# MyrtleSoftware/myrtlespeech

Hardware: AMD Instinct MI355X
Metric: audio-sec/s (RTF), DS2 5xBiLSTM-1024 encoder forward + CTC greedy, 80-feature 10 s clips @ batch 32/GPU (higher is better)
Workload: dtype f16x3 (f32 split in fp16 hi+lo, 3 fp16 MFMA passes, f32 acc: LSTM, projections, conv1/2, FC1; FC2/CTC/decode f32)

## Files before the change

### include/ms_hotpath.h

```cpp
#ifndef MS_HOTPATH_H
#define MS_HOTPATH_H

#include <stddef.h>
#include <stdint.h>

#ifdef __cplusplus
extern "C" {
#endif

#define MS_ABI_VERSION 4

enum {
  MS_OK = 0,
  MS_ERR_INVALID = 1,
  MS_ERR_HIP = 2,
  MS_ERR_WORKSPACE = 3,
  MS_ERR_TIMEOUT = 4,
  MS_ERR_UNSUPPORTED = 5
};

enum { MS_CELL_LSTM = 0, MS_CELL_GRU = 1, MS_CELL_RNN_TANH = 2, MS_CELL_HARD_LSTM = 3 };

enum { MS_ACT_NONE = 0, MS_ACT_CLAMP = 1  };

// ... 21 lines not shown
                           void* workspace, size_t workspace_bytes, void* stream);

size_t ms_maskconv_fwin_packed_bytes(int Cout, int KF, int KT);
int ms_maskconv_fwin_pack(const float* w, void* packed, int Cout, int KF, int KT, void* stream);
size_t ms_maskconv_fwin_workspace_bytes(int N, int Tin, int KF, int SF, int Fout);
int ms_maskconv_fwin_forward(const float* x, const int32_t* lens, const void* packed_w, const float* bias, float* y, int N,
                             int Fin, int Tin, int Cout, int Fout, int Tout, int KF, int KT, int SF, int ST, int DT,
                             int pad_f_l, int pad_t_l, int act, float act_lo, float act_hi, void* workspace,
                             size_t workspace_bytes, void* stream);

size_t ms_maskconv1d_gemm_packed_bytes(int Cout, int Cin, int KT);
int ms_maskconv1d_gemm_pack(const float* w, void* packed, int Cout, int Cin, int KT, void* stream);
size_t ms_maskconv1d_gemm_workspace_bytes(int N, int Cin, int Tout, int Cout, int KT);
int ms_maskconv1d_gemm_forward(const float* x, const int32_t* lens, const void* packed, const float* bias, float* y, int N,
                               int Cin, int Tin, int Cout, int Tout, int KT, int ST, int DT, int pad_l, int act,
                               float act_lo, float act_hi, void* workspace, size_t workspace_bytes, void* stream);

int ms_nct_to_tnc(const float* x, float* y, int N, int CF, int T, void* stream);

int ms_clamp(const float* x, float* y, size_t n, float lo, float hi, void* stream);


int ms_linear_forward(const float* x, const float* w, const float* bias, float* y, int M, int K, int N, int act,
                      float act_lo, float act_hi, void* stream);

#define MS_LINEAR_FEW_ROWS 1
size_t ms_linear_splitk_workspace_bytes(int M, int K, int N, int flags);
int ms_linear_splitk_forward(const float* x, const float* w, const float* bias, float* y, int M, int K, int N, int act,
                             float act_lo, float act_hi, int flags, void* workspace, size_t workspace_bytes, void* stream);

size_t ms_linear_split_workspace_bytes(int M, int K, int N);
int ms_linear_split_forward(const float* x, const float* w, const float* bias, float* y, int M, int K, int N, int act,
                            float act_lo, float act_hi, void* workspace, size_t workspace_bytes, void* stream);

size_t ms_linear_split_packed_bytes(int K, int N);
int ms_linear_split_pack(const float* w, void* packed, int K, int N, void* stream);
int ms_linear_split_forward_packed(const float* x, const void* packed_w, const float* bias, float* y, int M, int K, int N, int act,
                                   float act_lo, float act_hi, void* workspace, size_t workspace_bytes, void* stream);


int ms_lookahead_forward(const float* x, const float* w, float* y, int N, int F, int T, int ctx, long xs_n,
                         long xs_f, long xs_t, long ys_n, long ys_f, long ys_t, int act, float act_lo,
                         float act_hi, void* stream);

int ms_lookahead_window_forward(const float* x, const float* w, float* y, int N, int F, int T_in, int T_out, int ctx,
                                long xs_n, long xs_f, long xs_t, long ys_n, long ys_f, long ys_t, int act, float act_lo,
                                float act_hi, void* stream);


int ms_rnn_padded_hidden(int cell, int H, int ndir);
size_t ms_rnn_packed_bytes(int cell, int In, int H, int ndir);
int ms_rnn_pack(int cell, int In, int H, int ndir, const float* const* w_ih_host, const float* const* w_hh_host,
                const float* const* b_ih_host, const float* const* b_hh_host, void* packed, void* stream);

size_t ms_rnn_workspace_bytes(int cell, int T, int N, int In, int H, int ndir);

int ms_rnn_layer_forward(int cell, const void* packed, const float* x, const int32_t* lens, int max_len,
                         const float* h0, const float* c0, float* out, float* hn, float* cn, int T, int N, int In,
                         int H, int ndir, void* workspace, size_t workspace_bytes, void* stream);

enum { MS_RNN_X_PLANES_IN_WS = 1, MS_RNN_OUT_PLANES_TO_WS = 2, MS_RNN_PACKED_ROWS = 4, MS_RNN_HX_PREINIT = 4096,
       MS_RNN_RECURRENCE_ONLY = 8192, MS_RNN_TIMING_SKIP_PROJECTION = 8192 ,
       MS_RNN_PROJECTION_ONLY = 16384 };
int ms_rnn_layer_chains_planes(int cell, int H, int ndir);
int ms_rnn_hx_preinit(int cell, int T, int N, int In, int H, int ndir, int max_len, int nregions, void* workspace,
                      size_t workspace_bytes, void* stream);
int ms_rnn_layer_packs_rows(int cell, int T, int N, int In, int H, int ndir);
int ms_rnn_layer_forward_ex(int cell, const void* packed, const float* x, const int32_t* lens, int max_len,
                            const float* h0, const float* c0, float* out, float* hn, float* cn, int T, int N, int In,
                            int H, int ndir, int flags, void* workspace, size_t workspace_bytes, void* stream);

int ms_rnn_layer_is_wide(int cell, int H, int ndir, int N);
int ms_rnn_stack_overlap_ok(int cell, int T, int N, int In, int H, int ndir, int nl);
int ms_rnn_stack_forward(int cell, const void* const* packed_host, const float* x, const int32_t* lens, int max_len,
                         const float* h0, const float* c0, float* out, float* hn, float* cn, int T, int N, int In, int H, int ndir,
                         int nl, int segments, void* workspace, size_t workspace_bytes, void* stream);

int ms_rnn_status(const void* workspace, void* stream);

size_t ms_rnn_debug_offset(int cell, int T, int N, int In, int H, int ndir);

int ms_gemm_set_variant(int variant);

enum {
  MS_PROF_PROJECTION = 0, MS_PROF_RECURRENCE = 1, MS_PROF_GEMM_K_LARGE = 2, MS_PROF_GEMM_K_SMALL = 3, MS_PROF_CONV = 4,
  MS_PROF_LAYOUT = 5, MS_PROF_LINEAR = 6, MS_PROF_GREEDY = 7, MS_PROF_OTHER = 8
};
#define MS_PROF_KINDS 9
int ms_prof_enable(int on);
int ms_prof_read(float* out_ms_host, int* out_n_host);

int ms_clock_probe(unsigned long long* out_dev, int samples, int spacing_us, void* stream);

int ms_barrier_chain_probe(unsigned long long* out_dev, int steps, int threads, void* stream);


size_t ms_ctc_loss_workspace_bytes(int T, int N, int V, int S_max);

int ms_ctc_status(const void* workspace, void* stream);

#define MS_CTC_LOG_PROBS_IN 2
int ms_ctc_loss_forward(const float* logits, const int32_t* in_lens, const int32_t* targets,
                        const int32_t* tgt_offsets, const int32_t* tgt_lens, float* nll, float* reduced, int T,
                        int N, int V, int S_max, int blank, int reduction, int zero_infinity, void* workspace,
                        size_t workspace_bytes, void* stream);

int ms_log_softmax_axis(const float* x, float* y, int outer, int axis, int inner, void* stream);
int ms_log_softmax_axis_backward(const float* y, const float* g, float* gx, int outer, int axis, int inner, void* stream);

size_t ms_ctc_loss_backward_workspace_bytes(int T, int N, int V, int S_max);
int ms_ctc_loss_backward(const float* logits, const int32_t* in_lens, const int32_t* targets, const int32_t* tgt_offsets,
                         const int32_t* tgt_lens, const float* grad_nll, float* grad_logits, int T, int N, int V,
                         int S_max, int blank, int zero_infinity, void* workspace, size_t workspace_bytes, void* stream);


int ms_ctc_greedy_decode(const float* x, const int32_t* lens, int32_t* out_idx, int32_t* out_len, int T, int N,
                         int V, int blank, void* stream);

size_t ms_ctc_greedy_stream_state_bytes(int N);
int ms_ctc_greedy_stream_begin(void* state, int N, void* stream);
int ms_ctc_greedy_stream_step(const float* x, int rows, int n, int V, int blank, const int32_t* total_lens,
                              const int32_t* chunk_lens, int32_t* labels, int32_t* label_frames, int cap, int32_t* fresh,
                              void* state, int N, void* stream);


#define MS_CTC_ALIGN_BP_LDS_BYTES 98304
size_t ms_ctc_align_workspace_bytes(int T, int N, int V, int S_max);
int ms_ctc_align(const float* x, const int32_t* in_lens, const int32_t* targets, const int32_t* tgt_offsets,
                 const int32_t* tgt_lens, float* score, int32_t* frame_state, int32_t* token_start, int32_t* token_end,
                 float* token_logp, int T, int N, int V, int L_max, int blank, int flags, void* workspace,
                 size_t workspace_bytes, void* stream);


size_t ms_ctc_beam_workspace_bytes(int T, int N, int V, int beam_width);

int ms_ctc_beam_decode(const float* probs, const int32_t* lens, int32_t* out_idx, int32_t* out_len, int T, int N,
                       int V, int blank, int beam_width, float prune_threshold, int separator, const float* word_factor,
                       int t_begin, int t_end, const float* lm_factor, int finish, int32_t* beam_len,
                       int32_t* beam_idx, int32_t* beam_plen, void* workspace, size_t workspace_bytes,
                       void* stream);

int ms_ctc_beam_decode_rows(const float* probs, const int32_t* lens, int32_t* out_idx, int32_t* out_len, int T, int N,
                            int V, int blank, int beam_width, float prune_threshold, int separator,
                            const float* word_factor, int t_begin, int t_end, int row0, int rows_held,
                            const float* lm_factor, int finish, int32_t* beam_len, int32_t* beam_idx, int32_t* beam_plen,
                            void* workspace, size_t workspace_bytes, void* stream);


#define MS_NGRAM_MAX_ORDER 5

int ms_ngram_lm_table_check(const void* blob_host, size_t bytes);

int ms_ngram_lm_score(const void* table, const void* header_host, size_t table_bytes, const int32_t* prefixes,
                      const int32_t* prefix_lens, float* out, int P, int L, int separator, void* stream);

size_t ms_ctc_beam_lm_workspace_bytes(int T, int N, int V, int beam_width, int order);
int ms_ctc_beam_decode_lm(const float* probs, const int32_t* lens, int32_t* out_idx, int32_t* out_len, int T, int N,
                          int V, int blank, int beam_width, float prune_threshold, int separator,
                          const float* word_factor, int t_begin, int t_end, int row0, int rows_held, const void* lm_table,
                          const void* lm_header_host, size_t lm_table_bytes, int finish, int32_t* beam_len,
                          int32_t* beam_idx, int32_t* beam_plen, void* workspace, size_t workspace_bytes, void* stream);

int ms_ctc_beam_decode_ex(const float* probs, const int32_t* lens, int32_t* out_idx, int32_t* out_len, int T, int N,
                          int V, int blank, int beam_width, float prune_threshold, int separator,
                          const float* word_factor, int t_begin, int t_end, int row0, int rows_held,
                          const float* lm_factor, int finish, int32_t* beam_len, int32_t* beam_idx, int32_t* beam_plen,
// ... 62 lines not shown
```

### myrtlespeech_amd/_lib.py

```python
import ctypes
import os
import re
from ctypes import POINTER, c_char_p, c_double, c_float, c_int, c_int32, c_long, c_size_t, c_void_p

import torch

_HERE = os.path.dirname(os.path.abspath(__file__))
LIB_PATH = os.environ.get("MS_HOTPATH_LIB") or os.path.join(_HERE, "libms_hotpath.so")
HEADER_PATH = os.path.join(os.path.dirname(_HERE), "include", "ms_hotpath.h")

MS_OK = 0
ABI_VERSION = 4
ERR_NAMES = {1: "MS_ERR_INVALID", 2: "MS_ERR_HIP", 3: "MS_ERR_WORKSPACE", 4: "MS_ERR_TIMEOUT", 5: "MS_ERR_UNSUPPORTED"}

CELL_LSTM, CELL_GRU, CELL_RNN_TANH, CELL_HARD_LSTM = 0, 1, 2, 3
ACT_NONE, ACT_CLAMP = 0, 1
LINEAR_FEW_ROWS = 1
PROF_KINDS = 9

_P = c_void_p
_PP = POINTER(c_void_p)

SIGNATURES = {
    "ms_abi_version": (c_int, []),
    "ms_last_error": (c_char_p, []),
    "ms_mask_time_": (c_int, [_P, _P, c_int, c_int, c_int, _P]),
    "ms_maskconv_packed_bytes": (c_size_t, [c_int, c_int, c_int, c_int, c_int]),
    "ms_maskconv_pack": (c_int, [_P, _P, c_int, c_int, c_int, c_int, c_int, _P]),
    "ms_maskconv_forward": (c_int, [_P, _P, _P, _P, _P] + [c_int] * 17 + [c_float, c_float, _P]),
    "ms_maskconv_cl_packed_bytes": (c_size_t, [c_int, c_int, c_int, c_int]),
    "ms_maskconv_cl_pack": (c_int, [_P, _P, c_int, c_int, c_int, c_int, _P]),
    "ms_maskconv_cl_workspace_bytes": (c_size_t, [c_int, c_int, c_int, c_int]),
    "ms_maskconv_cl_forward": (c_int, [_P, _P, _P, _P, _P] + [c_int] * 16 + [c_float, c_float, _P, c_size_t, _P]),
    "ms_maskconv_fwin_packed_bytes": (c_size_t, [c_int, c_int, c_int]),
    "ms_maskconv_fwin_pack": (c_int, [_P, _P, c_int, c_int, c_int, _P]),
    "ms_maskconv_fwin_workspace_bytes": (c_size_t, [c_int, c_int, c_int, c_int, c_int]),
    "ms_maskconv_fwin_forward": (c_int, [_P, _P, _P, _P, _P] + [c_int] * 14 + [c_float, c_float, _P, c_size_t, _P]),
    "ms_maskconv1d_gemm_packed_bytes": (c_size_t, [c_int, c_int, c_int]),
    "ms_maskconv1d_gemm_pack": (c_int, [_P, _P, c_int, c_int, c_int, _P]),
    "ms_maskconv1d_gemm_workspace_bytes": (c_size_t, [c_int] * 5),
    "ms_maskconv1d_gemm_forward": (c_int, [_P, _P, _P, _P, _P] + [c_int] * 10 + [c_float, c_float, _P, c_size_t, _P]),
    "ms_nct_to_tnc": (c_int, [_P, _P, c_int, c_int, c_int, _P]),
    "ms_clamp": (c_int, [_P, _P, c_size_t, c_float, c_float, _P]),
    "ms_linear_forward": (c_int, [_P, _P, _P, _P, c_int, c_int, c_int, c_int, c_float, c_float, _P]),
    "ms_linear_splitk_workspace_bytes": (c_size_t, [c_int, c_int, c_int, c_int]),
    "ms_linear_splitk_forward": (c_int, [_P, _P, _P, _P, c_int, c_int, c_int, c_int, c_float, c_float, c_int, _P, c_size_t, _P]),
    "ms_linear_split_workspace_bytes": (c_size_t, [c_int, c_int, c_int]),
    "ms_linear_split_forward": (c_int, [_P, _P, _P, _P, c_int, c_int, c_int, c_int, c_float, c_float, _P, c_size_t, _P]),
    "ms_linear_split_packed_bytes": (c_size_t, [c_int, c_int]),
    "ms_linear_split_pack": (c_int, [_P, _P, c_int, c_int, _P]),
    "ms_linear_split_forward_packed": (c_int, [_P, _P, _P, _P, c_int, c_int, c_int, c_int, c_float, c_float, _P, c_size_t, _P]),
    "ms_lookahead_forward": (c_int, [_P, _P, _P, c_int, c_int, c_int, c_int] + [c_long] * 6 + [c_int, c_float, c_float, _P]),
    "ms_lookahead_window_forward": (c_int, [_P, _P, _P, c_int, c_int, c_int, c_int, c_int] + [c_long] * 6 + [c_int, c_float, c_float, _P]),
    "ms_rnn_packed_bytes": (c_size_t, [c_int, c_int, c_int, c_int]),
    "ms_ctc_status": (c_int, [_P, _P]),
    "ms_rnn_padded_hidden": (c_int, [c_int, c_int, c_int]),
    "ms_rnn_hx_preinit": (c_int, [c_int] * 8 + [_P, c_size_t, _P]),
    "ms_rnn_pack": (c_int, [c_int, c_int, c_int, c_int, _PP, _PP, _PP, _PP, _P, _P]),
    "ms_rnn_workspace_bytes": (c_size_t, [c_int] * 6),
    "ms_rnn_layer_forward": (c_int, [c_int, _P, _P, _P, c_int, _P, _P, _P, _P, _P] + [c_int] * 5 + [_P, c_size_t, _P]),
    "ms_rnn_layer_forward_ex": (c_int, [c_int, _P, _P, _P, c_int, _P, _P, _P, _P, _P] + [c_int] * 6 + [_P, c_size_t, _P]),
    "ms_rnn_layer_chains_planes": (c_int, [c_int, c_int, c_int]),
    "ms_rnn_layer_is_wide": (c_int, [c_int] * 4),
    "ms_rnn_stack_overlap_ok": (c_int, [c_int] * 7),
    "ms_rnn_stack_forward": (c_int, [c_int, _P, _P, _P, c_int, _P, _P, _P, _P, _P] + [c_int] * 7 + [_P, c_size_t, _P]),
    "ms_rnn_status": (c_int, [_P, _P]),
    "ms_rnn_debug_offset": (c_size_t, [c_int] * 6),
    "ms_rnn_layer_packs_rows": (c_int, [c_int] * 6),
    "ms_gemm_set_variant": (c_int, [c_int]),
    "ms_prof_enable": (c_int, [c_int]),
    "ms_prof_read": (c_int, [POINTER(c_float), POINTER(c_int)]),
    "ms_clock_probe": (c_int, [_P, c_int, c_int, _P]),
    "ms_barrier_chain_probe": (c_int, [_P, c_int, c_int, _P]),
    "ms_ctc_loss_workspace_bytes": (c_size_t, [c_int] * 4),
    "ms_ctc_loss_forward": (c_int, [_P] * 7 + [c_int] * 7 + [_P, c_size_t, _P]),
    "ms_log_softmax_axis": (c_int, [_P, _P, c_int, c_int, c_int, _P]),
    "ms_log_softmax_axis_backward": (c_int, [_P, _P, _P, c_int, c_int, c_int, _P]),
    "ms_ctc_loss_backward_workspace_bytes": (c_size_t, [c_int] * 4),
    "ms_ctc_loss_backward": (c_int, [_P] * 7 + [c_int] * 6 + [_P, c_size_t, _P]),
    "ms_ctc_greedy_decode": (c_int, [_P, _P, _P, _P, c_int, c_int, c_int, c_int, _P]),
    "ms_ctc_align_workspace_bytes": (c_size_t, [c_int] * 4),
    "ms_ctc_align": (c_int, [_P] * 10 + [c_int] * 6 + [_P, c_size_t, _P]),
    "ms_ctc_greedy_stream_state_bytes": (c_size_t, [c_int]),
    "ms_ctc_greedy_stream_begin": (c_int, [_P, c_int, _P]),
    "ms_ctc_greedy_stream_step": (c_int, [_P, c_int, c_int, c_int, c_int, _P, _P, _P, _P, c_int, _P, _P, c_int, _P]),
    "ms_embedding_forward": (c_int, [_P, _P, _P, c_int, c_int, c_int, _P]),
    "ms_rnnt_joint_forward": (c_int, [_P, _P, _P, _P, _P, _P, c_int, c_int, c_int, _P]),
    "ms_rnnt_topk": (c_int, [_P, _P, _P, c_int, c_int, c_int, _P]),
    "ms_ctc_beam_workspace_bytes": (c_size_t, [c_int] * 4),
    "ms_ctc_beam_decode": (c_int, [_P, _P, _P, _P, c_int, c_int, c_int, c_int, c_int, c_float, c_int, _P, c_int, c_int,
                                   _P, c_int, _P, _P, _P, _P, c_size_t, _P]),
    "ms_ctc_beam_decode_rows": (c_int, [_P, _P, _P, _P, c_int, c_int, c_int, c_int, c_int, c_float, c_int, _P, c_int, c_int,
                                        c_int, c_int, _P, c_int, _P, _P, _P, _P, c_size_t, _P]),
    "ms_ngram_lm_table_check": (c_int, [_P, c_size_t]),
    "ms_ngram_lm_score": (c_int, [_P, _P, c_size_t, _P, _P, _P, c_int, c_int, c_int, _P]),
    "ms_ctc_beam_lm_workspace_bytes": (c_size_t, [c_int] * 5),
    "ms_ctc_beam_decode_lm": (c_int, [_P, _P, _P, _P, c_int, c_int, c_int, c_int, c_int, c_float, c_int, _P, c_int, c_int,
                                      c_int, c_int, _P, _P, c_size_t, c_int, _P, _P, _P, _P, c_size_t, _P]),
    "ms_ctc_beam_decode_ex": (c_int, [_P, _P, _P, _P, c_int, c_int, c_int, c_int, c_int, c_float, c_int, _P, c_int, c_int,
                                      c_int, c_int, _P, c_int, _P, _P, _P, _P, c_size_t, _P, _P, _P, c_size_t, c_int, _P, _P]),
    "ms_rnnt_decode_workspace_bytes": (c_size_t, [c_int] * 10),
    "ms_rnnt_decode": (c_int, [_P, _P, _P, _PP, _PP, _PP, _PP, _P, _P, _P, _P, _P, _P] + [c_int] * 10 + [_P, c_size_t, _P]),
    "ms_rnnt_loss_lattice_bytes": (c_size_t, [c_int] * 3),
    "ms_rnnt_loss_workspace_bytes": (c_size_t, [c_int] * 4),
    "ms_rnnt_loss_forward": (c_int, [_P] * 6 + [c_int] * 5 + [_P, c_size_t, _P]),
    "ms_rnnt_loss_backward": (c_int, [_P] * 8 + [c_int] * 5 + [_P]),
    "ms_rnnt_score_lattice_bytes": (c_size_t, [c_int] * 3),
    "ms_rnnt_score_workspace_bytes": (c_size_t, [c_int] * 5),
    "ms_rnnt_score": (c_int, [_P] * 9 + [c_int] * 6 + [_P, c_size_t, _P]),
    "ms_mfcc_workspace_bytes": (c_size_t, [c_int] * 5),
    "ms_mfcc_forward": (c_int, [_P] * 7 + [c_int] * 7 + [c_float, _P, c_size_t, _P]),
    "ms_mfcc_legacy_forward": (c_int, [_P] * 7 + [c_int] * 8 + [c_double, _P]),
    "ms_standardize_workspace_bytes": (c_size_t, [c_int]),
    "ms_standardize_forward": (c_int, [_P, _P, _P, c_int, c_int, c_int, _P, c_size_t, _P]),
    "ms_context_frames_forward": (c_int, [_P, _P, _P, c_int, c_int, c_int, c_int, _P]),
    "ms_spec_augment_": (c_int, [_P, _P, _P] + [c_int] * 6 + [_P]),
}

_lib = None


def header_symbols():
    with open(HEADER_PATH) as f:
        text = re.sub(r"/\*.*?\*/", "", f.read(), flags=re.S)
    return sorted(set(re.findall(r"\b(ms_[a-z0-9_]+)\s*\(", text)))


def load():
    global _lib
    if _lib is None:
        if not os.path.exists(LIB_PATH):
            raise RuntimeError(
                f"{LIB_PATH} not found: build it with `python -c 'import __graft_entry__ as g; g.build()'` "
                "(or `make -C myrtlespeech_amd/csrc`). There is no CPU fallback."
            )
        lib = ctypes.CDLL(LIB_PATH)
        for name, (res, args) in SIGNATURES.items():
            fn = getattr(lib, name)
            fn.restype = res
            fn.argtypes = args
        got = lib.ms_abi_version()
        if got != ABI_VERSION:
            raise RuntimeError(f"{LIB_PATH} reports MS_ABI_VERSION {got}, this binding needs {ABI_VERSION}: rebuild the "
                               "library (`make -C myrtlespeech_amd/csrc`)")
        _lib = lib
    return _lib


def require_gpu():
    if not torch.cuda.is_available():
        raise RuntimeError("myrtlespeech_amd: a HIP device (MI355X) is required; there is no CPU fallback")

# ... 169 lines not shown
```

### myrtlespeech_amd/csrc/conv_cl.hip

```cpp
#include <algorithm>
#include <type_traits>

#include "common.h"

namespace {

typedef unsigned u32x4 __attribute__((ext_vector_type(4)));
typedef unsigned u32x2 __attribute__((ext_vector_type(2)));
typedef __bf16 bf16x8 __attribute__((ext_vector_type(8)));
typedef _Float16 f16x8 __attribute__((ext_vector_type(8)));

constexpr int CL_F = 2;

struct ClP {
  int N, Cin, Fin, Tin, Cout, Fout, Tout, KF, KT, SF, ST, DF, DT, pad_f, pad_t;
  int KG;
  int PW;
  int co_tiles;
  int act;
  float lo, hi;
  int FP;
};

__device__ __forceinline__ unsigned bf16b(float x) { return (unsigned)__builtin_bit_cast(unsigned short, (__bf16)x); }
// ... 70 lines not shown
      const int fin = (fo0 + f) * p.SF - p.pad_f + kf * p.DF;
      const bool frow = (fo0 + f) < p.Fout && (WIN || (fin >= 0 && fin < p.Fin));
      const size_t rbase = ((size_t)n * p.Fin + (frow && !WIN ? fin : 0)) * p.Tin;
      for (int i = tid; i < ngran; i += 256) {
        const int q = i / p.KG, kg = i - q * p.KG;
        const int tin = tin0 + q;
        u32x4 vh = {0u, 0u, 0u, 0u}, vl = {0u, 0u, 0u, 0u};
        if (frow && tin >= 0 && tin < len) {
          if (WIN) {
            const int boff = (int)((((size_t)n * p.Tin + tin) * p.FP + (size_t)(fo0 + f) * p.SF + kg * 8) * 2);
            vh = __builtin_amdgcn_raw_buffer_load_b128(xh_rsrc, boff, 0, 0);
            if (!F16) vl = __builtin_amdgcn_raw_buffer_load_b128(xl_rsrc, boff, 0, 0);
          } else {
            const size_t off = (rbase + tin) * p.Cin + kg * 8;
            vh = *reinterpret_cast<const u32x4*>(xh + off);
            if (!F16) vl = *reinterpret_cast<const u32x4*>(xl + off);
          }
        }
        *reinterpret_cast<u32x4*>(Ph + f * row_bytes + (kg * p.PW + q) * 16) = vh;
        if (!F16) *reinterpret_cast<u32x4*>(Pl + f * row_bytes + (kg * p.PW + q) * 16) = vl;
      }
    }
    const int taps_per_stage = (p.KT + 1) / 2;
    for (int kt0 = 0; kt0 < p.KT; kt0 += taps_per_stage) {
      const int ntap = min(taps_per_stage, p.KT - kt0);
      if (kt0 > 0) __syncthreads();
      {
        const int ng = ntap * p.KG * 32;
        for (int i = tid; i < ng; i += 256) {
          const int co = i & 31, rest = i >> 5;
          const size_t src = ((((size_t)kf * p.KT + kt0) * p.KG + rest) * cout_pad + tile * 32 + co) * 8;
          *reinterpret_cast<u32x4*>(Wh + i * 16) = *reinterpret_cast<const u32x4*>(wp + src);
          if (!F16) *reinterpret_cast<u32x4*>(Wl + i * 16) = *reinterpret_cast<const u32x4*>(wp + wplane + src);
        }
      }
      __syncthreads();
      for (int ktl = 0; ktl < ntap; ++ktl) {
        const int tq = (wt * 32 + l31) * p.ST + (kt0 + ktl) * p.DT;
        for (int s = 0; s < p.KG / 2; ++s) {
          const int kg = 2 * s + half;
          const int woff = ((ktl * p.KG + kg) * 32 + l31) * 16;
          const u32x4 ah = *reinterpret_cast<const u32x4*>(Wh + woff);
          u32x4 al = ah;
          if (!F16) al = *reinterpret_cast<const u32x4*>(Wl + woff);
#pragma unroll
          for (int f = 0; f < CL_F; ++f) {
            const int poff = (wf * CL_F + f) * row_bytes + (kg * p.PW + tq) * 16;
            const u32x4 bh = *reinterpret_cast<const u32x4*>(Ph + poff);
            if (F16) {
              acc[f] = __builtin_amdgcn_mfma_f32_32x32x16_f16(__builtin_bit_cast(f16x8, ah), __builtin_bit_cast(f16x8, bh), acc[f], 0, 0, 0);
            } else {
              const u32x4 bl = *reinterpret_cast<const u32x4*>(Pl + poff);
              acc[f] = ms::mfma_32x32x16<HM>(ah, bh, acc[f]);
              acc[f] = ms::mfma_32x32x16<HM>(al, bh, acc[f]);
              acc[f] = ms::mfma_32x32x16<HM>(ah, bl, acc[f]);
            }
          }
        }
      }
    }
    __syncthreads();
  }

  const int t = t0 + wt * 32 + l31;
  const float winv = scale_word[1];
  if (t < p.Tout) {
#pragma unroll
    for (int f = 0; f < CL_F; ++f) {
      const int fo = fo0 + wf * CL_F + f;
      if (fo >= p.Fout) continue;
#pragma unroll
      for (int r = 0; r < 16; ++r) {
        const int co = tile * 32 + ms::mfma32_row(r, lane);
        if (co < p.Cout) {
          float v = acc[f][r] * winv + (bias ? bias[co] : 0.f);
          if (p.act == MS_ACT_CLAMP) v = fminf(fmaxf(v, p.lo), p.hi);
          y[(((size_t)n * p.Cout + co) * p.Fout + fo) * p.Tout + t] = v;
        }
      }
    }
  }
}


constexpr int SH_RB = 12;
constexpr int SH_KT = 11;

template <int P>
__global__ __launch_bounds__(256, 1) void maskconv_cl_short_kernel(const unsigned short* __restrict__ xh,
                                                                   const unsigned short* __restrict__ xl,
                                                                   const int32_t* __restrict__ lens,
                                                                   const unsigned short* __restrict__ wp,
                                                                   const float* __restrict__ bias, float* __restrict__ y, ClP p,
                                                                   int RB, int RIN, const float* __restrict__ scale_word) {
  constexpr bool F16 = ms::prec_one_plane(P), HM = P == ms::PREC_F16X3;
  const float winv = scale_word[1];
  extern __shared__ __attribute__((aligned(16))) char lds[];
  const int tid = threadIdx.x, lane = tid & 63, wave = __builtin_amdgcn_readfirstlane(tid >> 6);
  const int c16 = lane & 15, q = lane >> 4;
  const int fo0 = blockIdx.x * RB, cb = blockIdx.y, n = blockIdx.z;
  const int PW = p.PW;
  const int row_bytes = PW * 64;
  char* Ph = lds;
  char* Pl = lds + (size_t)RIN * row_bytes;
  const int len = lens ? min(lens[n], p.Tin) : p.Tin;
  const int fin_lo = fo0 * p.SF - p.pad_f;

  for (int i = tid; i < RIN * PW * 4; i += 256) {
    const int kg = i & 3, rq = i >> 2;
    const int r = rq / PW, fq = rq - r * PW;
    const int fin = fin_lo + r, tin = fq - p.pad_t;
    u32x4 vh = {0u, 0u, 0u, 0u}, vl = {0u, 0u, 0u, 0u};
    if (fin >= 0 && fin < p.Fin && tin >= 0 && tin < len) {
      const size_t off = (((size_t)n * p.Fin + fin) * p.Tin + tin) * 32 + kg * 8;
      vh = *reinterpret_cast<const u32x4*>(xh + off);
      if (!F16) vl = *reinterpret_cast<const u32x4*>(xl + off);
    }
    *reinterpret_cast<u32x4*>(Ph + r * row_bytes + fq * 64 + kg * 16) = vh;
    if (!F16) *reinterpret_cast<u32x4*>(Pl + r * row_bytes + fq * 64 + kg * 16) = vl;
  }
  __syncthreads();

  ms::f32x4 acc[SH_RB];
#pragma unroll
  for (int i = 0; i < SH_RB; ++i) acc[i] = ms::f32x4{0.f, 0.f, 0.f, 0.f};
  const int cout_pad = p.co_tiles * 32;
  const size_t wplane = (size_t)p.KF * p.KT * 4 * cout_pad * 8;
  const unsigned short* wa = wp + (size_t)q * cout_pad * 8 + (cb * 16 + c16) * 8;
  const size_t tap_stride = (size_t)4 * cout_pad * 8;
  u32x4 fh[2][SH_KT], fl[2][SH_KT];
  auto load_row = [&](auto set, int kf) {
#pragma unroll
    for (int kt = 0; kt < SH_KT; ++kt)
      if (kt < p.KT) {
        const unsigned short* src = wa + (size_t)(kf * p.KT + kt) * tap_stride;
        fh[set][kt] = *reinterpret_cast<const u32x4*>(src);
        if (!F16) fl[set][kt] = *reinterpret_cast<const u32x4*>(src + wplane);
      }
  };
  auto compute_row = [&](auto set, int kf) {
#pragma unroll
    for (int i = 0; i < SH_RB; ++i) {
      const int fo = fo0 + i;
      const int fin = fo * p.SF - p.pad_f + kf * p.DF;
      if (i < RB && fo < p.Fout && fin >= 0 && fin < p.Fin) {
        const int rbase = (fin - fin_lo) * row_bytes + c16 * 64 + q * 16;
#pragma unroll
        for (int kt = 0; kt < SH_KT; ++kt)
          if (kt < p.KT) {
            const u32x4 bh = *reinterpret_cast<const u32x4*>(Ph + rbase + kt * 64);
            if (F16) {
              acc[i] = __builtin_amdgcn_mfma_f32_16x16x32_f16(__builtin_bit_cast(f16x8, fh[set][kt]), __builtin_bit_cast(f16x8, bh), acc[i], 0, 0, 0);
            } else {
              const u32x4 bl = *reinterpret_cast<const u32x4*>(Pl + rbase + kt * 64);
              acc[i] = ms::mfma_16x16x32<HM>(fh[set][kt], bh, acc[i]);
              acc[i] = ms::mfma_16x16x32<HM>(fl[set][kt], bh, acc[i]);
              acc[i] = ms::mfma_16x16x32<HM>(fh[set][kt], bl, acc[i]);
            }
          }
      }
    }
  };
  constexpr std::integral_constant<int, 0> S0{};
  constexpr std::integral_constant<int, 1> S1{};
  if (wave < p.KF) load_row(S0, wave);
  for (int kf = wave; kf < p.KF; kf += 8) {
// ... 44 lines not shown
  }
  return 0;
}

__global__ void nchw_to_cl_split_kernel(const float* __restrict__ x, unsigned short* __restrict__ hi,
                                        unsigned short* __restrict__ lo, int C, int F, int T, int prec) {
  __shared__ float tile[32][33];
  const int n = blockIdx.z / F, f = blockIdx.z % F;
  const int t0 = blockIdx.x * 32, c0 = blockIdx.y * 32;
  const int tx = threadIdx.x, ty = threadIdx.y;
  for (int i = ty; i < 32; i += 8) {
    const int c = c0 + i, t = t0 + tx;
    tile[i][tx] = (c < C && t < T) ? x[(((size_t)n * C + c) * F + f) * T + t] : 0.f;
  }
  __syncthreads();
  for (int i = ty; i < 32; i += 8) {
    const int t = t0 + i, c = c0 + tx;
    if (t < T && c < C) {
      const float v = tile[tx][i];
      const size_t o = (((size_t)n * F + f) * T + t) * C + c;
      unsigned h, l;
      split_by_prec(v, prec, h, l);
      hi[o] = (unsigned short)h;
      if (prec != ms::PREC_F16) lo[o] = (unsigned short)l;
    }
  }
}

__global__ void ft_to_tf_split_kernel(const float* __restrict__ x, unsigned short* __restrict__ hi,
                                      unsigned short* __restrict__ lo, int Fin, int T, int FP, int pad, int prec) {
  __shared__ float tile[32][33];
  const int n = blockIdx.z;
  const int t0 = blockIdx.x * 32, j0 = blockIdx.y * 32;
  const int tx = threadIdx.x, ty = threadIdx.y;
  for (int i = ty; i < 32; i += 8) {
    const int fidx = j0 + i - pad, t = t0 + tx;
    tile[i][tx] = (fidx >= 0 && fidx < Fin && t < T) ? x[((size_t)n * Fin + fidx) * T + t] : 0.f;
  }
  __syncthreads();
  for (int i = ty; i < 32; i += 8) {
    const int t = t0 + i, j = j0 + tx;
    if (t < T && j < FP) {
      const float v = tile[tx][i];
      const size_t o = ((size_t)n * T + t) * FP + j;
      unsigned h, l;
      split_by_prec(v, prec, h, l);
      hi[o] = (unsigned short)h;
      if (prec != ms::PREC_F16) lo[o] = (unsigned short)l;
    }
  }
}

__global__ void conv_fwin_pack_kernel(const float* __restrict__ w, unsigned short* __restrict__ packed, int Cout, int KF,
                                      int KT, int KG, int cout_pad, int prec, const float* __restrict__ scale_word) {
  const size_t plane = (size_t)KT * KG * cout_pad * 8;
  const float wscale = scale_word[0];
  for (size_t i = (size_t)blockIdx.x * blockDim.x + threadIdx.x; i < plane; i += (size_t)gridDim.x * blockDim.x) {
    const int e = i & 7;
    const int co = (i >> 3) % cout_pad;
    const int kg = (i / ((size_t)8 * cout_pad)) % KG;
    const int kt = i / ((size_t)8 * cout_pad * KG);
    const int kf = kg * 8 + e;
    float x = 0.f;
    if (co < Cout && kf < KF) x = w[((size_t)co * KF + kf) * KT + kt] * wscale;
    unsigned h, l;
    split_by_prec(x, prec, h, l);
    packed[i] = (unsigned short)h;
    packed[plane + i] = (unsigned short)l;
  }
}

int conv_cl_plan(ClP& p, size_t* lds) {
  const size_t wbytes = (size_t)2 * ((p.KT + 1) / 2) * p.KG * 32 * 16;
  if ((long)p.N * p.co_tiles > 65535) return 0;
  for (int wf : {p.Tout <= 48 ? 4 : 1, 1}) {
    const int tt = 128 / wf, rf = CL_F * wf;
    p.PW = (tt - 1) * p.ST + (p.KT - 1) * p.DT + 1;
    *lds = (size_t)2 * rf * p.KG * p.PW * 16 + wbytes;
    if (*lds <= 160 * 1024 && ms::cdiv(p.Fout, rf) <= 65535) return wf;
  }
  return 0;
}

template <bool WIN>
int conv_cl_launch(const ClP& p, int wf, size_t lds, const unsigned short* xh, const unsigned short* xl, const int32_t* lens,
                   const void* packed_w, const float* bias, float* y, hipStream_t stream, const float* scale_word) {
  static ms::DeviceOnce attr_once;
  if (attr_once.need()) {
#define MS_CL_ATTR(PP)                                                                                                                     \
    MS_HIP(hipFuncSetAttribute((const void*)maskconv_cl_kernel<PP, WIN, 1>, hipFuncAttributeMaxDynamicSharedMemorySize, 160 * 1024));   \
    MS_HIP(hipFuncSetAttribute((const void*)maskconv_cl_kernel<PP, WIN, 4>, hipFuncAttributeMaxDynamicSharedMemorySize, 160 * 1024));
    MS_CL_ATTR(ms::PREC_BF16X3) MS_CL_ATTR(ms::PREC_F16) MS_CL_ATTR(ms::PREC_F16X3)
#undef MS_CL_ATTR
    attr_once.done();
  }
  const int prec = ms::split_mode();
  const int tt = 128 / wf, rf = CL_F * wf;
  dim3 grid(ms::cdiv(p.Tout, tt), ms::cdiv(p.Fout, rf), p.N * p.co_tiles);
  const unsigned short* wq = (const unsigned short*)packed_w;
#define MS_CL_LAUNCH(WF_)                                                                                                             \
  if (prec == ms::PREC_F16) hipLaunchKernelGGL((maskconv_cl_kernel<ms::PREC_F16, WIN, WF_>), grid, dim3(256), lds, stream, xh, xl, lens, wq, bias, y, p, scale_word); \
  else if (prec == ms::PREC_F16X3) hipLaunchKernelGGL((maskconv_cl_kernel<ms::PREC_F16X3, WIN, WF_>), grid, dim3(256), lds, stream, xh, xl, lens, wq, bias, y, p, scale_word); \
  else hipLaunchKernelGGL((maskconv_cl_kernel<ms::PREC_BF16X3, WIN, WF_>), grid, dim3(256), lds, stream, xh, xl, lens, wq, bias, y, p, scale_word);
  if (wf == 4) { MS_CL_LAUNCH(4) } else { MS_CL_LAUNCH(1) }
#undef MS_CL_LAUNCH
  MS_LAUNCH_CHECK();
  return MS_OK;
}

inline int fwin_kfp(int KF) { return ms::cdiv(KF, 16) * 16; }
inline int fwin_fp(int KF, int SF, int Fout) { return ms::cdiv((Fout - 1) * SF + fwin_kfp(KF), 32) * 32; }

}

static size_t fwin_plane_bytes(int Cout, int KF, int KT) {
  return ms::align_up((size_t)2 * KT * (fwin_kfp(KF) / 8) * (ms::cdiv(Cout, 32) * 32) * 8 * sizeof(unsigned short), 256);
}
extern "C" size_t ms_maskconv_fwin_packed_bytes(int Cout, int KF, int KT) {
  if (Cout <= 0 || KF <= 0 || KT <= 0) return 0;
  return fwin_plane_bytes(Cout, KF, KT) + 256;
}

extern "C" int ms_maskconv_fwin_pack(const float* w, void* packed, int Cout, int KF, int KT, void* stream) {
  MS_REQUIRE(w && packed, "null pointer");
  MS_REQUIRE(Cout > 0 && KF > 0 && KT > 0, "bad shape");
  const int cout_pad = ms::cdiv(Cout, 32) * 32, KG = fwin_kfp(KF) / 8;
  const size_t plane = (size_t)KT * KG * cout_pad * 8;
  const int blocks = (int)std::min<size_t>((plane + 255) / 256, 2048);
  float* scale_word = (float*)((char*)packed + fwin_plane_bytes(Cout, KF, KT));
  const int rc = ms::weight_scale_launch(w, (size_t)Cout * KF * KT, scale_word, ms::split_mode(), (hipStream_t)stream);
  if (rc != MS_OK) return rc;
  hipLaunchKernelGGL(conv_fwin_pack_kernel, dim3(blocks), dim3(256), 0, (hipStream_t)stream, w, (unsigned short*)packed, Cout,
                     KF, KT, KG, cout_pad, ms::split_mode(), scale_word);
  MS_LAUNCH_CHECK();
  return MS_OK;
}

extern "C" size_t ms_maskconv_fwin_workspace_bytes(int N, int Tin, int KF, int SF, int Fout) {
  if (N <= 0 || Tin <= 0 || KF <= 0 || SF <= 0 || Fout <= 0) return 0;
  return ms::align_up((size_t)N * Tin * fwin_fp(KF, SF, Fout) * 4, 256);
}

extern "C" int ms_maskconv_fwin_forward(const float* x, const int32_t* lens, const void* packed_w, const float* bias, float* y,
                                        int N, int Fin, int Tin, int Cout, int Fout, int Tout, int KF, int KT, int SF, int ST,
                                        int DT, int pad_f_l, int pad_t_l, int act, float act_lo, float act_hi, void* workspace,
                                        size_t workspace_bytes, void* stream_) {
  ms::ProfScope prof_span(MS_PROF_CONV, (hipStream_t)stream_);
  MS_REQUIRE(x && packed_w && y && workspace, "null pointer");
  MS_REQUIRE(N > 0 && Fin > 0 && Tin > 0 && Cout > 0 && Fout > 0 && Tout > 0, "bad shape");
  MS_REQUIRE(KF > 0 && KT > 0 && SF > 0 && ST > 0 && DT > 0 && pad_f_l >= 0 && pad_t_l >= 0, "bad kernel");
  MS_REQUIRE(SF % 2 == 0, "feature stride must be even (4-byte aligned window loads)");
  MS_REQUIRE(act == MS_ACT_NONE || act == MS_ACT_CLAMP, "bad act");
  if (workspace_bytes < ms_maskconv_fwin_workspace_bytes(N, Tin, KF, SF, Fout)) {
    ms::set_error("ms_maskconv_fwin_forward: workspace too small");
    return MS_ERR_WORKSPACE;
  }
  hipStream_t stream = (hipStream_t)stream_;
  ClP p;
  p.N = N; p.Cin = fwin_kfp(KF); p.Fin = 1; p.Tin = Tin; p.Cout = Cout; p.Fout = Fout; p.Tout = Tout; p.KF = 1; p.KT = KT;
  p.SF = SF; p.ST = ST; p.DF = 1; p.DT = DT; p.pad_f = 0; p.pad_t = pad_t_l; p.KG = p.Cin / 8;
  p.co_tiles = ms::cdiv(Cout, 32);
  p.act = act; p.lo = act_lo; p.hi = act_hi;
  p.FP = fwin_fp(KF, SF, Fout);
  size_t lds = 0;
  const int wf = conv_cl_plan(p, &lds);
  if (wf == 0 || (size_t)N * Tin * p.FP * 2 >= ((size_t)1 << 31)) {
// ... 16 lines not shown
}
extern "C" size_t ms_maskconv_cl_packed_bytes(int Cout, int Cin, int KF, int KT) {
  if (Cout <= 0 || Cin <= 0 || Cin % 16 || KF <= 0 || KT <= 0) return 0;
  return cl_plane_bytes(Cout, Cin, KF, KT) + 256;
}

extern "C" int ms_maskconv_cl_pack(const float* w, void* packed, int Cout, int Cin, int KF, int KT, void* stream) {
  MS_REQUIRE(w && packed, "null pointer");
  MS_REQUIRE(Cout > 0 && Cin > 0 && Cin % 16 == 0 && KF > 0 && KT > 0, "bad shape (Cin must be a multiple of 16)");
  const int cout_pad = ms::cdiv(Cout, 32) * 32;
  const size_t plane = (size_t)KF * KT * (Cin / 8) * cout_pad * 8;
  const int blocks = (int)std::min<size_t>((plane + 255) / 256, 2048);
  float* scale_word = (float*)((char*)packed + cl_plane_bytes(Cout, Cin, KF, KT));
  const int rc = ms::weight_scale_launch(w, (size_t)Cout * Cin * KF * KT, scale_word, ms::split_mode(), (hipStream_t)stream);
  if (rc != MS_OK) return rc;
  hipLaunchKernelGGL(conv_cl_pack_kernel, dim3(blocks), dim3(256), 0, (hipStream_t)stream, w, (unsigned short*)packed, Cout,
                     Cin, KF, KT, cout_pad, ms::split_mode(), scale_word);
  MS_LAUNCH_CHECK();
  return MS_OK;
}

extern "C" size_t ms_maskconv_cl_workspace_bytes(int N, int Cin, int Fin, int Tin) {
  if (N <= 0 || Cin <= 0 || Fin <= 0 || Tin <= 0) return 0;
  return ms::align_up((size_t)N * Cin * Fin * Tin * 4, 256);
}

extern "C" int ms_maskconv_cl_forward(const float* x, const int32_t* lens, const void* packed_w, const float* bias, float* y,
                                      int N, int Cin, int Fin, int Tin, int Cout, int Fout, int Tout, int KF, int KT,
                                      int SF, int ST, int DF, int DT, int pad_f_l, int pad_t_l, int act, float act_lo,
                                      float act_hi, void* workspace, size_t workspace_bytes, void* stream_) {
  ms::ProfScope prof_span(MS_PROF_CONV, (hipStream_t)stream_);
  MS_REQUIRE(x && packed_w && y && workspace, "null pointer");
  MS_REQUIRE(N > 0 && Cin > 0 && Cin % 16 == 0 && Fin > 0 && Tin > 0 && Cout > 0 && Fout > 0 && Tout > 0, "bad shape");
  MS_REQUIRE(KF > 0 && KT > 0 && SF > 0 && ST > 0 && DF > 0 && DT > 0 && pad_f_l >= 0 && pad_t_l >= 0, "bad kernel");
  MS_REQUIRE(act == MS_ACT_NONE || act == MS_ACT_CLAMP, "bad act");
  if (workspace_bytes < ms_maskconv_cl_workspace_bytes(N, Cin, Fin, Tin)) {
    ms::set_error("ms_maskconv_cl_forward: workspace too small");
    return MS_ERR_WORKSPACE;
  }
  hipStream_t stream = (hipStream_t)stream_;
  ClP p;
  p.N = N; p.Cin = Cin; p.Fin = Fin; p.Tin = Tin; p.Cout = Cout; p.Fout = Fout; p.Tout = Tout; p.KF = KF; p.KT = KT;
  p.SF = SF; p.ST = ST; p.DF = DF; p.DT = DT; p.pad_f = pad_f_l; p.pad_t = pad_t_l; p.KG = Cin / 8;
  p.co_tiles = ms::cdiv(Cout, 32);
  p.act = act; p.lo = act_lo; p.hi = act_hi;
  p.FP = 0;
  size_t lds = 0;
  const int wf = conv_cl_plan(p, &lds);
  if (wf == 0) {
    ms::set_error("ms_maskconv_cl_forward: shape outside the LDS / grid budget");
    return MS_ERR_UNSUPPORTED;
  }
  const float* scale_word = (const float*)((const char*)packed_w + cl_plane_bytes(Cout, Cin, KF, KT));
  unsigned short* xh = (unsigned short*)workspace;
  unsigned short* xl = xh + (size_t)N * Cin * Fin * Tin;
  MS_REQUIRE(N * Fin <= 65535, "N*Fin exceeds grid limits");
  const int prec = ms::split_mode();
  const bool f16 = prec == ms::PREC_F16;
  hipLaunchKernelGGL(nchw_to_cl_split_kernel, dim3(ms::cdiv(Tin, 32), ms::cdiv(Cin, 32), N * Fin), dim3(32, 8), 0, stream, x,
                     xh, xl, Cin, Fin, Tin, prec);
  MS_LAUNCH_CHECK();
  {
    int RB = 0, RIN = 0;
    size_t slds = 0;
    if (conv_cl_short_plan(p, f16, &RB, &RIN, &slds)) {
      static ms::DeviceOnce attr_once;
      if (attr_once.need()) {
        MS_HIP(hipFuncSetAttribute((const void*)maskconv_cl_short_kernel<ms::PREC_BF16X3>, hipFuncAttributeMaxDynamicSharedMemorySize, 160 * 1024));
        MS_HIP(hipFuncSetAttribute((const void*)maskconv_cl_short_kernel<ms::PREC_F16>, hipFuncAttributeMaxDynamicSharedMemorySize, 160 * 1024));
        MS_HIP(hipFuncSetAttribute((const void*)maskconv_cl_short_kernel<ms::PREC_F16X3>, hipFuncAttributeMaxDynamicSharedMemorySize, 160 * 1024));
        attr_once.done();
      }
      ClP ps = p;
      ps.PW = Tout + KT - 1;
      const dim3 grid(ms::cdiv(Fout, RB), ms::cdiv(Cout, 16), N);
      const unsigned short* wq = (const unsigned short*)packed_w;
      auto kern = prec == ms::PREC_F16 ? maskconv_cl_short_kernel<ms::PREC_F16>
                  : prec == ms::PREC_F16X3 ? maskconv_cl_short_kernel<ms::PREC_F16X3> : maskconv_cl_short_kernel<ms::PREC_BF16X3>;
      hipLaunchKernelGGL(kern, grid, dim3(256), slds, stream, xh, xl, lens, wq, bias, y, ps, RB, RIN, scale_word);
      MS_LAUNCH_CHECK();
      return MS_OK;
    }
  }
  return conv_cl_launch<false>(p, wf, lds, xh, xl, lens, packed_w, bias, y, stream, scale_word);
}
```

Measured before the change: 27490.

## Add register-staged pipelined channels-last masked conv kernel with sliding row window

Adds a new channels-last masked convolution kernel that keeps a sliding window of input frequency rows in LDS and prefetches the next row and next weight half-stage into registers while MFMAs run on the current ones. It double-buffers fragment reads from LDS against MFMA issue using sched barriers. It uses less LDS, launching with two blocks per CU, and becomes the default path when shapes fit (stride-1 dilation in frequency, no FP padding). The aim is to hide global load latency and raise occupancy relative to the original whole-tile staging kernel. In exchange it adds more synchronization per tap stage and higher register pressure.

```diff
diff --git a/include/ms_hotpath.h b/include/ms_hotpath.h
--- a/include/ms_hotpath.h
+++ b/include/ms_hotpath.h
@@ -127,6 +127,10 @@
 
 int ms_gemm_set_variant(int variant);
 
+int ms_conv_cl_set_variant(int variant);
+long ms_conv_cl_pipelined_launches(void);
+int ms_maskconv_cl_tile_plan(int N, int Cin, int Cout, int Fout, int Tout, int KT, int SF, int ST, int DF, int DT);
+
 enum {
   MS_PROF_PROJECTION = 0, MS_PROF_RECURRENCE = 1, MS_PROF_GEMM_K_LARGE = 2, MS_PROF_GEMM_K_SMALL = 3, MS_PROF_CONV = 4,
   MS_PROF_LAYOUT = 5, MS_PROF_LINEAR = 6, MS_PROF_GREEDY = 7, MS_PROF_OTHER = 8
diff --git a/myrtlespeech_amd/_lib.py b/myrtlespeech_amd/_lib.py
--- a/myrtlespeech_amd/_lib.py
+++ b/myrtlespeech_amd/_lib.py
@@ -68,6 +68,9 @@
     "ms_rnn_debug_offset": (c_size_t, [c_int] * 6),
     "ms_rnn_layer_packs_rows": (c_int, [c_int] * 6),
     "ms_gemm_set_variant": (c_int, [c_int]),
+    "ms_conv_cl_set_variant": (c_int, [c_int]),
+    "ms_conv_cl_pipelined_launches": (c_long, []),
+    "ms_maskconv_cl_tile_plan": (c_int, [c_int] * 10),
     "ms_prof_enable": (c_int, [c_int]),
     "ms_prof_read": (c_int, [POINTER(c_float), POINTER(c_int)]),
     "ms_clock_probe": (c_int, [_P, c_int, c_int, _P]),
diff --git a/myrtlespeech_amd/csrc/conv_cl.hip b/myrtlespeech_amd/csrc/conv_cl.hip
--- a/myrtlespeech_amd/csrc/conv_cl.hip
+++ b/myrtlespeech_amd/csrc/conv_cl.hip
@@ -176,6 +176,197 @@
   }
 }
 
+constexpr int PIPE_ROW_MAX = 5;
+constexpr int PIPE_W_MAX = 6;
+constexpr size_t PIPE_LDS_MAX = 80 * 1024;
+
+template <int P>
+__global__ __launch_bounds__(256, 2) void maskconv_cl_pipe_kernel(const unsigned short* __restrict__ xh,
+                                                                  const unsigned short* __restrict__ xl,
+                                                                  const int32_t* __restrict__ lens,
+                                                                  const unsigned short* __restrict__ wp,
+                                                                  const float* __restrict__ bias, float* __restrict__ y, ClP p,
+                                                                  int NW, const float* __restrict__ scale_word) {
+  constexpr bool F16 = ms::prec_one_plane(P), HM = P == ms::PREC_F16X3;
+  constexpr int TT = 128;
+  extern __shared__ __attribute__((aligned(16))) char lds[];
+  const int row_bytes = p.KG * p.PW * 16;
+  const int taps_per_stage = (p.KT + 1) / 2;
+  const int wtap = p.KG * 32 * 16;
+  char* Ph = lds;
+  char* Pl = lds + NW * row_bytes;
+  char* Wh = lds + 2 * NW * row_bytes;
+  char* Wl = Wh + taps_per_stage * wtap;
+
+  const int tid = threadIdx.x, lane = tid & 63, wave = tid >> 6;
+  const int l31 = lane & 31, half = lane >> 5;
+  const int t0 = blockIdx.x * TT;
+  const int fo0 = blockIdx.y * CL_F;
+  const int n = blockIdx.z / p.co_tiles, tile = blockIdx.z % p.co_tiles;
+  const int len = lens ? min(lens[n], p.Tin) : p.Tin;
+  const int cout_pad = p.co_tiles * 32;
+  const size_t wplane = (size_t)p.KF * p.KT * p.KG * cout_pad * 8;
+
+  ms::f32x16 acc[CL_F];
+#pragma unroll
+  for (int f = 0; f < CL_F; ++f)
+#pragma unroll
+    for (int r = 0; r < 16; ++r) acc[f][r] = 0.f;
+
+  const int tin0 = t0 * p.ST - p.pad_t;
+  const int ngran = p.KG * p.PW;
+  int rsrc[PIPE_ROW_MAX], rdst[PIPE_ROW_MAX];
+#pragma unroll
+  for (int k = 0; k < PIPE_ROW_MAX; ++k) {
+    const int i = tid + 256 * k;
+    const int q = i / p.KG, kg = i - q * p.KG;
+    const int tin = tin0 + q;
+    rdst[k] = i < ngran ? (kg * p.PW + q) * 16 : -1;
+    rsrc[k] = (i < ngran && tin >= 0 && tin < len) ? tin * p.Cin + kg * 8 : -1;
+  }
+  const int wsrc = ((tid >> 5) * cout_pad + tile * 32 + (tid & 31)) * 8;
+  const int fin0 = fo0 * p.SF - p.pad_f;
+
+  u32x4 rh[PIPE_ROW_MAX], rl[PIPE_ROW_MAX], fh[PIPE_W_MAX], fl[PIPE_W_MAX];
+  bool row_ok = false;
+  auto load_row = [&](int j) {
+    const int fin = fin0 + j;
+    row_ok = fin >= 0 && fin < p.Fin;
+    const size_t rbase = ((size_t)n * p.Fin + (row_ok ? fin : 0)) * p.Tin * p.Cin;
+#pragma unroll
+    for (int k = 0; k < PIPE_ROW_MAX; ++k)
+      if (256 * k < ngran) {
+        const int off = max(rsrc[k], 0);
+        rh[k] = *reinterpret_cast<const u32x4*>(xh + rbase + off);
+        if (!F16) rl[k] = *reinterpret_cast<const u32x4*>(xl + rbase + off);
+      }
+  };
+  auto store_row = [&](int slot) {
+#pragma unroll
+    for (int k = 0; k < PIPE_ROW_MAX; ++k)
+      if (256 * k < ngran) {
+        const bool keep = row_ok && rsrc[k] >= 0;
+        const u32x4 zero = {0u, 0u, 0u, 0u};
+        if (rdst[k] >= 0) {
+          *reinterpret_cast<u32x4*>(Ph + slot * row_bytes + rdst[k]) = keep ? rh[k] : zero;
+          if (!F16) *reinterpret_cast<u32x4*>(Pl + slot * row_bytes + rdst[k]) = keep ? rl[k] : zero;
+        }
+      }
+  };
+  auto load_w = [&](int kf, int kt0, int ntap) {
+    const int ng = ntap * p.KG * 32;
+    const unsigned short* src = wp + (size_t)(kf * p.KT + kt0) * p.KG * cout_pad * 8;
+#pragma unroll
+    for (int k = 0; k < PIPE_W_MAX; ++k)
+      if (256 * k < ng) {
+        const int off = tid + 256 * k < ng ? wsrc + k * 64 * cout_pad : 0;
+        fh[k] = *reinterpret_cast<const u32x4*>(src + off);
+        if (!F16) fl[k] = *reinterpret_cast<const u32x4*>(src + wplane + off);
+      }
+  };
+  auto store_w = [&](int ntap) {
+    const int ng = ntap * p.KG * 32;
+#pragma unroll
+    for (int k = 0; k < PIPE_W_MAX; ++k)
+      if (tid + 256 * k < ng) {
+        *reinterpret_cast<u32x4*>(Wh + (tid + 256 * k) * 16) = fh[k];
+        if (!F16) *reinterpret_cast<u32x4*>(Wl + (tid + 256 * k) * 16) = fl[k];
+      }
+  };
+
+  for (int j = 0; j < NW; ++j) {
+    load_row(j);
+    store_row(j);
+  }
+  load_w(0, 0, min(taps_per_stage, p.KT));
+  store_w(min(taps_per_stage, p.KT));
+  __syncthreads();
+
+  const int nhalf = p.KT > taps_per_stage ? 2 : 1;
+  int slot0 = 0;
+  for (int kf = 0; kf < p.KF; ++kf) {
+    const int slot1 = slot0 == 0 ? NW - 1 : slot0 - 1;
+    for (int h = 0; h < nhalf; ++h) {
+      const int kt0 = h * taps_per_stage;
+      const int ntap = min(taps_per_stage, p.KT - kt0);
+      const bool last_half = h == nhalf - 1;
+      const int nkf = last_half ? kf + 1 : kf, nkt0 = last_half ? 0 : taps_per_stage;
+      const int nntap = min(taps_per_stage, p.KT - nkt0);
+      const bool more = nkf < p.KF;
+      if (more) load_w(nkf, nkt0, nntap);
+      if (h == 0 && kf + 1 < p.KF) load_row(kf + NW);
+
+      const int nstep = ntap * (p.KG / 2);
+      int rk = 0, rs = 0;
+      auto read_frags = [&](u32x4& ah, u32x4& al, u32x4 (&bh)[CL_F], u32x4 (&bl)[CL_F]) {
+        const int kg = 2 * rs + half;
+        const int woff = ((rk * p.KG + kg) * 32 + l31) * 16;
+        const int tq = (wave * 32 + l31) * p.ST + (kt0 + rk) * p.DT;
+        ah = *reinterpret_cast<const u32x4*>(Wh + woff);
+        if (!F16) al = *reinterpret_cast<const u32x4*>(Wl + woff);
+#pragma unroll
+        for (int f = 0; f < CL_F; ++f) {
+          const int poff = (f == 0 ? slot0 : slot1) * row_bytes + (kg * p.PW + tq) * 16;
+          bh[f] = *reinterpret_cast<const u32x4*>(Ph + poff);
+          if (!F16) bl[f] = *reinterpret_cast<const u32x4*>(Pl + poff);
+        }
+        if (++rs == p.KG / 2) { rs = 0; if (++rk == ntap) rk = 0; }
+      };
+      auto mfma_step = [&](const u32x4& ah, const u32x4& al, const u32x4 (&bh)[CL_F], const u32x4 (&bl)[CL_F]) {
+#pragma unroll
+        for (int f = 0; f < CL_F; ++f) {
+          if (F16) {
+            acc[f] = __builtin_amdgcn_mfma_f32_32x32x16_f16(__builtin_bit_cast(f16x8, ah), __builtin_bit_cast(f16x8, bh[f]), acc[f], 0, 0, 0);
+          } else {
+            acc[f] = ms::mfma_32x32x16<HM>(ah, bh[f], acc[f]);
+            acc[f] = ms::mfma_32x32x16<HM>(al, bh[f], acc[f]);
+            acc[f] = ms::mfma_32x32x16<HM>(ah, bl[f], acc[f]);
+          }
+        }
+      };
+      u32x4 ah0, al0, bh0[CL_F], bl0[CL_F], ah1, al1, bh1[CL_F], bl1[CL_F];
+      read_frags(ah0, al0, bh0, bl0);
+      for (int it = 0; it < nstep; it += 2) {
+        read_frags(ah1, al1, bh1, bl1);
+        __builtin_amdgcn_sched_barrier(0);
+        mfma_step(ah0, al0, bh0, bl0);
+        __builtin_amdgcn_sched_barrier(0);
+        if (it + 1 >= nstep) break;
+        read_frags(ah0, al0, bh0, bl0);
+        __builtin_amdgcn_sched_barrier(0);
+        mfma_step(ah1, al1, bh1, bl1);
+        __builtin_amdgcn_sched_barrier(0);
+      }
+      if (!more) break;
+      __builtin_amdgcn_s_waitcnt(0x0070);
+      __syncthreads();
+      store_w(nntap);
+      if (last_half) store_row(slot0);
+      __syncthreads();
+    }
+    slot0 = slot0 + 1 == NW ? 0 : slot0 + 1;
+  }
+
+  const int t = t0 + wave * 32 + l31;
+  const float winv = scale_word[1];
+  if (t < p.Tout) {
+#pragma unroll
+    for (int f = 0; f < CL_F; ++f) {
+      const int fo = fo0 + f;
+      if (fo >= p.Fout) continue;
+#pragma unroll
+      for (int r = 0; r < 16; ++r) {
+        const int co = tile * 32 + ms::mfma32_row(r, lane);
+        if (co < p.Cout) {
+          float v = acc[f][r] * winv + (bias ? bias[co] : 0.f);
+          if (p.act == MS_ACT_CLAMP) v = fminf(fmaxf(v, p.lo), p.hi);
+          y[(((size_t)n * p.Cout + co) * p.Fout + fo) * p.Tout + t] = v;
+        }
+      }
+    }
+  }
+}
+
 
 constexpr int SH_RB = 12;
 constexpr int SH_KT = 11;
@@ -386,6 +577,40 @@
   return 0;
 }
 
+std::atomic<int> g_conv_cl_variant{0};
+std::atomic<long> g_conv_cl_pipe_launches{0};
+
+int conv_cl_pipe_plan(const ClP& p, int wf, int* NW, size_t* lds) {
+  if (wf != 1 || p.FP != 0 || p.DF != 1) return 0;
+  const int nw = (CL_F - 1) * p.SF + 1;
+  const size_t ngran = (size_t)p.KG * p.PW, wgran = (size_t)((p.KT + 1) / 2) * p.KG * 32;
+  const size_t bytes = 2 * nw * ngran * 16 + 2 * wgran * 16;
+  if (ngran > PIPE_ROW_MAX * 256 || wgran > PIPE_W_MAX * 256 || bytes > PIPE_LDS_MAX) return 0;
+  *NW = nw;
+  *lds = bytes;
+  return 1;
+}
+
+int conv_cl_pipe_launch(const ClP& p, int NW, size_t lds, const unsigned short* xh, const unsigned short* xl, const int32_t* lens,
+                        const void* packed_w, const float* bias, float* y, hipStream_t stream, const float* scale_word) {
+  static ms::DeviceOnce attr_once;
+  if (attr_once.need()) {
+    MS_HIP(hipFuncSetAttribute((const void*)maskconv_cl_pipe_kernel<ms::PREC_BF16X3>, hipFuncAttributeMaxDynamicSharedMemorySize, (int)PIPE_LDS_MAX));
+    MS_HIP(hipFuncSetAttribute((const void*)maskconv_cl_pipe_kernel<ms::PREC_F16>, hipFuncAttributeMaxDynamicSharedMemorySize, (int)PIPE_LDS_MAX));
+    MS_HIP(hipFuncSetAttribute((const void*)maskconv_cl_pipe_kernel<ms::PREC_F16X3>, hipFuncAttributeMaxDynamicSharedMemorySize, (int)PIPE_LDS_MAX));
+    attr_once.done();
+  }
+  const int prec = ms::split_mode();
+  const dim3 grid(ms::cdiv(p.Tout, 128), ms::cdiv(p.Fout, CL_F), p.N * p.co_tiles);
+  const unsigned short* wq = (const unsigned short*)packed_w;
+  auto kern = prec == ms::PREC_F16 ? maskconv_cl_pipe_kernel<ms::PREC_F16>
+              : prec == ms::PREC_F16X3 ? maskconv_cl_pipe_kernel<ms::PREC_F16X3> : maskconv_cl_pipe_kernel<ms::PREC_BF16X3>;
+  hipLaunchKernelGGL(kern, grid, dim3(256), lds, stream, xh, xl, lens, wq, bias, y, p, NW, scale_word);
+  MS_LAUNCH_CHECK();
+  g_conv_cl_pipe_launches.fetch_add(1, std::memory_order_relaxed);
+  return MS_OK;
+}
+
 template <bool WIN>
 int conv_cl_launch(const ClP& p, int wf, size_t lds, const unsigned short* xh, const unsigned short* xl, const int32_t* lens,
                    const void* packed_w, const float* bias, float* y, hipStream_t stream, const float* scale_word) {
@@ -568,5 +793,31 @@
       return MS_OK;
     }
   }
+  {
+    int NW = 0;
+    size_t plds = 0;
+    if (g_conv_cl_variant.load(std::memory_order_relaxed) != 1 && conv_cl_pipe_plan(p, wf, &NW, &plds))
+      return conv_cl_pipe_launch(p, NW, plds, xh, xl, lens, packed_w, bias, y, stream, scale_word);
+  }
   return conv_cl_launch<false>(p, wf, lds, xh, xl, lens, packed_w, bias, y, stream, scale_word);
 }
+
+extern "C" int ms_conv_cl_set_variant(int v) {
+  g_conv_cl_variant.store(v, std::memory_order_relaxed);
+  return MS_OK;
+}
+
+extern "C" long ms_conv_cl_pipelined_launches(void) { return g_conv_cl_pipe_launches.load(std::memory_order_relaxed); }
+
+extern "C" int ms_maskconv_cl_tile_plan(int N, int Cin, int Cout, int Fout, int Tout, int KT, int SF, int ST, int DF, int DT) {
+  if (N <= 0 || Cin <= 0 || Cin % 16 || Cout <= 0 || Fout <= 0 || Tout <= 0 || KT <= 0 || SF <= 0 || ST <= 0 || DF <= 0 || DT <= 0)
+    return 0;
+  ClP p{};
+  p.N = N; p.Cin = Cin; p.Cout = Cout; p.Fout = Fout; p.Tout = Tout; p.KT = KT; p.SF = SF; p.ST = ST; p.DF = DF; p.DT = DT;
+  p.KG = Cin / 8;
+  p.co_tiles = ms::cdiv(Cout, 32);
+  size_t lds = 0;
+  const int wf = conv_cl_plan(p, &lds);
+  int NW = 0;
+  return conv_cl_pipe_plan(p, wf, &NW, &lds) ? 2 : wf;
+}
```

Result: no change. 27340 (median of 2 runs) (-0.5%).
